# line/open-universe

Hardware: AMD Instinct MI355X
Metric: real_time_factor (audio s / wall s), UNIVERSE++ 16 kHz 8-step enhance (higher is better)
Workload: dtype f32; 1 GPU; UNIVERSE++ 16 kHz, 8 diffusion steps, batch=1 utterance(s) of 4 s per GPU per step; network=PP16, n_diffusion_steps=8, batch_per_gpu=1, samples_per_utterance=64000, launches_per_enhance=414

## Files before the change

open-universe_amd/csrc/ou_api.cpp:

```cpp
#include <hip/hip_runtime.h>

#include <cmath>
#include <cstdio>
#include <cstdlib>
#include <cstring>
#include <map>
#include <string>
#include <vector>

#include "../../include/ouniverse.h"
#include "../../include/ouniverse_tuning.h"
#include "ou_kernels.h"
#include "ou_model.h"

using namespace ou;

namespace {
thread_local std::string g_last_error;
constexpr int kMaxSteps = 256;
constexpr size_t kProfSlots = 32768;
constexpr float kInvSqrt2 = 0.70710678118654752440f;
constexpr size_t align256(size_t bytes) { return (bytes + 255) & ~size_t(255); }

struct TensorRef {
  size_t off;
  int C, T;
};
struct Options {
  int dbg = 0, xcd_map = -1, conv_direct = 5, fuse = -1, fuse_nc = 0, rate_small = 1, fuse_upfir = 1, block3 = 0, d4_fir = 1,
      d4_force = 0, d4_short = 1, d2_wk = 0, wino = 1, d2_map = -1, unfuse64 = 0, preact = 1;
  int gru_v = 2, gru_bmax = 0, gru_ts = 0, gru_upw = 0, gru_backoff = 0, gru_agent = -1, gru_dbg = 0;
  int split = -1;
  int dbg_dec0_under_gru = 0;
  int tile_prefetch = 1;
  int trace = 0, no_overlap = 0, ts = 0, deep_factor = 8, mask_fused = 1, split_wino = 1, d2_tile_rule = 1;
  int ens_share = 1;
  double tile_min = -1.0;
  std::string chain_ts;
};
}

struct ou_packer {
  Model m;
  std::map<std::string, HostTensor> sd;
  std::vector<float> blob;
  std::string err;
};

struct ou_handle {
  Model m;
  const float* W = nullptr;
  int device = 0;
  int num_cu = 256;
  std::string err;
  std::map<std::string, TensorRef> tensors;
  int n_launch = 0, n_conv = 0;
  int cond_B = 0, cond_T = 0;
  bool trace = false;
  Options opt;
  NormMode norm;
  std::string plan_with_options;
  int last_cfg = -1;
  long long* tstamps = nullptr;
  std::map<size_t, float> alphas;
  hipStream_t aux[3] = {nullptr, nullptr, nullptr};
  std::vector<hipEvent_t> events;
  size_t ev_used = 0;
  bool overlap = true;
  int force_cfg = -1, force_sc = 0;
  bool profile = false;
  struct ProfRec { double flops, bytes; int cfg; };
  std::vector<ProfRec> prof;
  size_t prof_used = 0;
  unsigned long long* prof_dev = nullptr;
  struct WsRec { const void* ws; size_t bytes; int B, T; };
  std::vector<WsRec> ws_ready;
  int gru_agent_stores = 0;
  int lanes = 1, lane = 0;
  int lane_max_b = 0;
  struct NoiseSource {
    bool on = false;
    unsigned long long seed = 0;
    std::vector<unsigned long long> streams;
    float* scratch = nullptr;
    size_t scratch_bytes = 0;
  } noise_src;
  double plane_per_sample = 0.0, wav_plane_per_sample = 0.0;
  bool ws_ok(const void* ws, size_t bytes, int B, int T) const {
    (void)T;
    for (const WsRec& r : ws_ready)
      if (r.ws == ws) return r.B == B && r.bytes <= bytes;
    return false;
  }
};

namespace {

int fail(ou_handle* h, int code, const std::string& msg) {
  if (h) h->err = msg;
  g_last_error = msg;
  return code;
}

struct Tensor {
  float* p = nullptr;
  int C = 0, T = 0;
};

struct OptDesc {
  const char* key;
  int Options::*ip;
  double Options::*dp;
  bool experiments_only;
  const char* doc;
};
const OptDesc kOptions[] = {
    {"conv_direct", &Options::conv_direct, nullptr, false, "kernel generations the conv launcher may use (0 .. 5, ConvArgs::direct)"},
    {"split", &Options::split, nullptr, false, "-1 rule / 0 never / 1 wherever possible: conv_split_kernel (bf16-split operands)"},
    {"split_wino", &Options::split_wino, nullptr, false, "experiments build: 0 = the plain bf16-split kernel also where its minimal-filtering form would take the layer"},
    {"wino", &Options::wino, nullptr, false, "0: never the minimal-filtering (Winograd / Cook-Toom) kernel variants"},
    {"fuse", &Options::fuse, nullptr, false, "-1 cost model / 0 never / 2 / 3: depth of the fused ConvBlock body (conv_chain kernels)"},
    {"fuse_nc", &Options::fuse_nc, nullptr, false, "128 / 256: columns per tile of the fused ConvBlock body (0: launcher's choice)"},
    {"fuse_upfir", &Options::fuse_upfir, nullptr, false, "0: up-path anti-alias FIR always as its own pass"},
    {"rate_small", &Options::rate_small, nullptr, false, "0: outermost rate-change convs on the generic kernels (no rate_down / rate_up)"},
    {"preact", &Options::preact, nullptr, false, "0: every PReLU in its consumer's operand path (ConvArgs::out_act never set)"},
    {"unfuse64", &Options::unfuse64, nullptr, false, "1: 64-channel ConvBlock bodies as three split-K launches"},
    {"block3", &Options::block3, nullptr, false, "1: the three body convs of a deep-level ConvBlock in one launch (experiments build only)"},
    {"xcd_map", &Options::xcd_map, nullptr, false, "block -> tile mapping of the LDS-tiled conv kernel (-1: launcher's choice)"},
    {"d2_map", &Options::d2_map, nullptr, false, "block -> tile mapping of the wide-load split-K kernels (-1: launcher's choice)"},
    {"d2_tile_rule", &Options::d2_tile_rule, nullptr, false, "0: round 5's 64- vs 32-column rule of the wide-load split-K kernels (ignores that only 64-column tiles have minimal filtering)"},
    {"d2_wk", &Options::d2_wk, nullptr, false, "4 / 8: K slices of conv_direct2_kernel (0: launcher's rule)"},
    {"d4_fir", &Options::d4_fir, nullptr, false, "0: up convs with a fusable FIR stay on the first-generation fused kernel"},
    {"d4_short", &Options::d4_short, nullptr, false, "0: the 401-frame levels at batch 1 stay on the first-generation kernels"},
    {"d4_force", &Options::d4_force, nullptr, false, "10 TM + log2(WK): that conv_direct4 tile shape wherever a layer admits it"},
    {"tile_min", nullptr, &Options::tile_min, false, "wave tiles per SIMD from which the no-split-K kernels take a layer (< 0: 1.2)"},
    {"tile_prefetch", &Options::tile_prefetch, nullptr, false, "0: no LDS prefetch of the epilogue operand in conv_direct3_kernel"},
    {"deep_factor", &Options::deep_factor, nullptr, false, "blocks of 64 x 128 per CU up to which a layer counts as 'deep' (split-K kernels)"},
    {"mask_fused", &Options::mask_fused, nullptr, false, "ragged batches: 0 = a separate tail-mask launch after EVERY producer (reference form of the masks)"},
    {"gru_v", &Options::gru_v, nullptr, false, "2 ring kernel / 1 polling-wave kernel (experiments build)"},
    {"gru_bmax", &Options::gru_bmax, nullptr, false, "cap on the utterances per GRU launch (forces the chunked path)"},
    {"gru_upw", &Options::gru_upw, nullptr, false, "hidden units per workgroup of the ring kernel (0: from the batch size)"},
    {"gru_backoff", &Options::gru_backoff, nullptr, false, "poll back-off experiments of the ring kernel (0: none)"},
    {"gru_agent_stores", &Options::gru_agent, nullptr, false, "-1 handle's mode / 0 plain / 1 agent-scope publishes"},
    {"gru_dbg", &Options::gru_dbg, nullptr, false, "bit 0 no republish safety net, bit 1 system-scope publishes, bit 2 FAULT INJECTION (tests)"},
    {"gru_ts", &Options::gru_ts, nullptr, false, "1: per-wave cycle stamps of the GRU kernel into the end of the workspace (tuning)"},
    {"ts", &Options::ts, nullptr, false, "1: per-wave phase stamps in ou_bench_conv (tuning)"},
    {"trace", &Options::trace, nullptr, false, "1: one line per conv launch on stderr"},
    {"no_overlap", &Options::no_overlap, nullptr, false, "1: no side streams inside a call (every kernel alone on the device)"},
    {"ens_share", &Options::ens_share, nullptr, false, "ou_enhance_ensemble: 1 = conditioner once over the B inputs, its results replicated; 0 = over all E * B rows"},
    {"dbg", &Options::dbg, nullptr, true, "phase ablation switches of the conv kernels: WRONG results by design"},
    {"dbg_dec0", &Options::dbg_dec0_under_gru, nullptr, true, "first decoder block under the GRU: upper-bound measurement, WRONG results"},
};
constexpr int kNumOptions = (int)(sizeof(kOptions) / sizeof(kOptions[0]));
const OptDesc* find_option(const char* key) {
  for (int i = 0; i < kNumOptions; i++)
    if (std::strcmp(kOptions[i].key, key) == 0) return &kOptions[i];
  return nullptr;
}

struct Runner {
  ou_handle* h;
  Options env;
  char* base;
  size_t cap;
  size_t off = 0;
  bool dry;
  hipStream_t st;
  hipStream_t main_st;
  int B;
  hipError_t herr = hipSuccess;
  bool oom = false;
  const char* where = "";
  size_t max_plane = 0;
  bool mel_scale_preset = false;
  bool ragged = false;
  const int* lens_dev = nullptr;
  const RowInfo* rows_dev = nullptr;
  LevelSpec lv;
  int level_T[kMaxLenLevels] = {0};
  unsigned* status_words = nullptr;
  unsigned long long* block3_bar = nullptr;
  int gru_area_rows = 0;
  bool gru_shared = false;

  Runner(ou_handle* h_, void* ws, size_t cap_, bool dry_, hipStream_t st_, int B_)
      : h(h_), env(h_->opt), base((char*)ws), cap(cap_), dry(dry_), st(st_), main_st(st_), B(B_) {
#ifndef OU_EXPERIMENTS
    env.dbg = 0; env.dbg_dec0_under_gru = 0;
#endif
  }
  static Runner conditioner_of(const Runner& r, int Bc) {
    Runner c(r.h, r.base, r.cap, false, r.st, Bc);
    c.status_words = r.status_words;
    c.block3_bar = r.block3_bar;
    c.gru_area_rows = r.B;
    c.off = r.off;
    c.mel_scale_preset = r.mel_scale_preset;
    c.lv = r.lv;
    for (int l = 0; l < kMaxLenLevels; l++) c.level_T[l] = r.level_T[l];
    return c;
  }
  void set_ragged(const int* lens, const RowInfo* rows) {
    ragged = true;
    lens_dev = lens;
    rows_dev = rows;
  }

  bool ok() const { return herr == hipSuccess && !oom; }
  template <class F>
  void launch(const char* w, F&& enqueue) {
    if (dry || !ok()) return;
    chk(enqueue(), w);
  }

  float* alloc_raw(size_t floats) {
// ... 2470 lines not shown
```

open-universe_amd/csrc/ou_conv_direct4.hip:

```cpp
#include "ou_kernels.h"
#include "ou_internal.h"
#include "ou_dev.h"

#include <cmath>
#include <cstdlib>
#include <type_traits>

namespace ou {

typedef float f32x4acc __attribute__((ext_vector_type(4)));

template <int R, int TM, int WN, int WK, int D>
__global__ __launch_bounds__(64 * WN * WK) void conv_direct4_kernel(ConvArgs p) {
  constexpr int TN = 4, LPS = 2 * R, BM = 16 * TM, NW = WN * WK, EP = 68;
  static_assert(WN == 1 || WK == 1, "a block is either WN column tiles or WK slices of the reduction");
  static_assert(TM >= 1 && TM <= 4, "16 .. 64-row tiles");
  static_assert(D * LPS <= 60, "loads in flight must fit vmcnt");
  static_assert(D == 2 || D == 4, "ring depth");
  typedef float f32x3 __attribute__((ext_vector_type(3)));
  typedef typename std::conditional<TM == 4, f32x4, typename std::conditional<TM == 3, f32x3,
          typename std::conditional<TM == 2, f32x2, float>::type>::type>::type avec;
  extern __shared__ __attribute__((aligned(16))) float smem[];
  const int tid = threadIdx.x, lane = tid & 63;
  const int wv = __builtin_amdgcn_readfirstlane(tid >> 6);
  const int wn = WK == 1 ? wv : 0, wk = WK == 1 ? 0 : wv;
  const int L = blockIdx.x, q8 = L >> 3;
  int rg, cidx;
  if (p.xcd_map == 1) {
    const int gm8 = (p.grid_m + 7) >> 3;
    rg = (q8 % gm8) * 8 + (L & 7);
    cidx = q8 / gm8;
  } else {
    rg = q8 % p.grid_m;
    cidx = (q8 / p.grid_m) * 8 + (L & 7);
  }
  const int b = cidx / p.grid_n, chunk = cidx - b * p.grid_n;
  const int n0 = (chunk * WN + wn) * 64, m0 = rg * BM;
  if (b >= p.B || rg >= p.grid_m) return;
  if (WK == 1 && n0 >= p.Nq) return;
  if (p.prof && tid == 0) atomicMin(p.prof + (blockIdx.x & 15), (unsigned long long)__builtin_amdgcn_s_memrealtime());
  const int l15 = lane & 15, kk = lane >> 4;
  const int Tin = p.Tin, Mp = p.Mp, CK = p.CK, lck = 31 - __clz(CK);
  const float alpha = p.act ? p.alpha_val : 1.0f;
  const u32x4 rx = direct_desc(p.x + (size_t)b * p.Cin * Tin, (unsigned)p.Cin * (unsigned)Tin * 4u);
  const u32x4 rw = direct_desc(p.w, (unsigned)p.Cin * (unsigned)R * (unsigned)Mp * 4u);
  const int avo = (kk * Mp + m0 + TM * l15) * 4;
  const int c0 = n0 + TN * l15;
  const int bvo = c0 < p.Nq ? (kk * Tin + c0 * R) * 4 : (int)0x80000000;

  const int NS = (p.Cin >> 2) / WK;
  avec a4[D][R];
  f32x4 b4[D][R];
#pragma unroll
  for (int d0 = 0; d0 < D; d0++)
#pragma unroll
    for (int k = 0; k < R; k++) {
      if constexpr (TM == 4) a4[d0][k] = f32x4{0.f, 0.f, 0.f, 0.f};
      else if constexpr (TM == 3) a4[d0][k] = f32x3{0.f, 0.f, 0.f};
      else if constexpr (TM == 2) a4[d0][k] = f32x2{0.f, 0.f};
      else a4[d0][k] = 0.f;
      b4[d0][k] = f32x4{0.f, 0.f, 0.f, 0.f};
    }
  f32x4acc acc[TM][TN];
#pragma unroll
  for (int i = 0; i < TM; i++)
#pragma unroll
    for (int j = 0; j < TN; j++) acc[i][j] = f32x4acc{0.f, 0.f, 0.f, 0.f};

#define OU_ISSUE(g_, d)                                                                                                  \
  {                                                                                                                      \
    const int c4 = (wk + WK * (g_)) * 4;                                                                                 \
    const int wrow = ((c4 >> lck) * R) * CK + (c4 & (CK - 1));                   \
    const int xso = c4 * Tin * 4;                                                                                        \
    _Pragma("unroll") for (int k = 0; k < R; k++) {                                                                      \
      if constexpr (TM == 4)                                                                                             \
        asm volatile("buffer_load_dwordx4 %0, %1, %2, %3 offen" : "+v"(a4[d][k]) : "v"(avo), "s"(rw), "s"((wrow + k * CK) * Mp * 4)); \
      else if constexpr (TM == 3)                                                                                        \
        asm volatile("buffer_load_dwordx3 %0, %1, %2, %3 offen" : "+v"(a4[d][k]) : "v"(avo), "s"(rw), "s"((wrow + k * CK) * Mp * 4)); \
      else if constexpr (TM == 2)                                                                                        \
        asm volatile("buffer_load_dwordx2 %0, %1, %2, %3 offen" : "+v"(a4[d][k]) : "v"(avo), "s"(rw), "s"((wrow + k * CK) * Mp * 4)); \
      else                                                                                                               \
        asm volatile("buffer_load_dword %0, %1, %2, %3 offen" : "+v"(a4[d][k]) : "v"(avo), "s"(rw), "s"((wrow + k * CK) * Mp * 4)); \
    }                                                                                                                    \
    _Pragma("unroll") for (int k = 0; k < R; k++)                                                                        \
      asm volatile("buffer_load_dwordx4 %0, %1, %2, %3 offen offset:%4" : "+v"(b4[d][k]) : "v"(bvo), "s"(rx), "s"(xso), "n"(16 * k)); \
  }
#define OU_MMA(d, out)                                                                                                   \
  {                                                                                                                      \
    asm volatile("s_waitcnt vmcnt(%0)" ::"n"((out) * LPS));                                                              \
    _Pragma("unroll") for (int k = 0; k < R; k++) { asm volatile("" : "+v"(a4[d][k])); asm volatile("" : "+v"(b4[d][k])); } \
    float X[4 * R];                                                                                                      \
    _Pragma("unroll") for (int k = 0; k < R; k++) {                                                                      \
      X[4 * k + 0] = b4[d][k].x; X[4 * k + 1] = b4[d][k].y; X[4 * k + 2] = b4[d][k].z; X[4 * k + 3] = b4[d][k].w;        \
    }                                                                                                                    \
    _Pragma("unroll") for (int e = 0; e < 4 * R; e++) X[e] = X[e] >= 0.f ? X[e] : alpha * X[e];                          \
    _Pragma("unroll") for (int k = 0; k < R; k++)                                                                        \
      _Pragma("unroll") for (int i = 0; i < TM; i++) {                                                                   \
        float av;                                                                                                        \
        if constexpr (TM == 1) av = a4[d][k]; else av = a4[d][k][i];                                                     \
        _Pragma("unroll") for (int j = 0; j < TN; j++)                                                                   \
          acc[i][j] = __builtin_amdgcn_mfma_f32_16x16x4f32(av, X[j * R + k], acc[i][j], 0, 0, 0);                        \
      }                                                                                                                  \
  }
  const bool ts_on = p.tstamps != nullptr;
  long long tc0 = 0, tc1 = 0, tc2 = 0, tr0 = 0;
  if (ts_on) { tr0 = (long long)__builtin_amdgcn_s_memrealtime(); tc0 = __builtin_readcyclecounter(); }
  if constexpr (D == 4) {
    OU_ISSUE(0, 0); OU_ISSUE(1, 1); OU_ISSUE(2, 2); OU_ISSUE(3, 3);
    if (ts_on) tc1 = __builtin_readcyclecounter();
    const int NR = NS / 4;
    for (int r = 0; r + 1 < NR; r++) {
      const int g = r * 4;
      OU_MMA(0, 3); OU_ISSUE(g + 4, 0);
      OU_MMA(1, 3); OU_ISSUE(g + 5, 1);
      OU_MMA(2, 3); OU_ISSUE(g + 6, 2);
      OU_MMA(3, 3); OU_ISSUE(g + 7, 3);
    }
    OU_MMA(0, 3); OU_MMA(1, 2); OU_MMA(2, 1); OU_MMA(3, 0);
  } else {
    OU_ISSUE(0, 0); OU_ISSUE(1, 1);
    if (ts_on) tc1 = __builtin_readcyclecounter();
    const int NR = NS / 2;
    for (int r = 0; r + 1 < NR; r++) {
      const int g = r * 2;
      OU_MMA(0, 1); OU_ISSUE(g + 2, 0);
      OU_MMA(1, 1); OU_ISSUE(g + 3, 1);
    }
    OU_MMA(0, 1); OU_MMA(1, 0);
  }
  if (ts_on) tc2 = __builtin_readcyclecounter();
#undef OU_ISSUE
#undef OU_MMA

  float* Ew = smem + (size_t)wv * BM * EP;
#pragma unroll
  for (int i = 0; i < TM; i++)
#pragma unroll
    for (int r = 0; r < 4; r++)
      *reinterpret_cast<f32x4*>(&Ew[(TM * (4 * kk + r) + i) * EP + 4 * l15]) =
          f32x4{acc[i][0][r], acc[i][1][r], acc[i][2][r], acc[i][3][r]};
  if constexpr (WK > 1) asm volatile("s_waitcnt lgkmcnt(0)\n\ts_barrier" ::: "memory");
  else asm volatile("s_waitcnt lgkmcnt(0)" ::: "memory");

  const int rt = WK == 1 ? lane : tid;
  constexpr int RNT = WK == 1 ? 64 : 64 * WK;
  const float* Er = WK == 1 ? Ew : smem;
  const float* filmb = p.film ? p.film + (size_t)b * p.film_bstride : nullptr;
  const size_t ybase = (size_t)b * p.Cout * p.Tout;
  const float insc = p.in_scale ? p.in_scale[b] : 1.0f;
  const int nvalid = p.Nq - n0;
  const int rlen = ragged_len(p.lens, b);
  if (p.up == 1) {
    constexpr int NQ = BM * 16, QPT = (NQ + RNT - 1) / RNT;
#pragma unroll
    for (int u = 0; u < QPT; u++) {
      const int e = rt + u * RNT;
      if (NQ % RNT != 0 && e >= NQ) break;
      const int row = e >> 4, cq = (e & 15) * 4;
      const int m = m0 + row;
      if (m >= p.M || cq >= nvalid) continue;
      const size_t idx = ybase + (size_t)m * p.Tout + n0 + cq;
      const bool full = cq + 4 <= nvalid;
      f32x4 ad = {0.f, 0.f, 0.f, 0.f}, rs = {0.f, 0.f, 0.f, 0.f};
      if (full) {
        if (p.add) ad = *reinterpret_cast<const f32x4u*>(p.add + idx);
        if (p.res) rs = *reinterpret_cast<const f32x4u*>(p.res + idx);
      } else {
#pragma unroll
        for (int s = 0; s < 4; s++) {
          if (p.add && cq + s < nvalid) ad[s] = p.add[idx + s];
          if (p.res && cq + s < nvalid) rs[s] = p.res[idx + s];
        }
      }
      f32x4 v = *reinterpret_cast<const f32x4*>(&Er[row * EP + cq]);
#pragma unroll
      for (int k = 1; k < WK; k++) v += *reinterpret_cast<const f32x4*>(&Er[(k * BM + row) * EP + cq]);
      if (p.in_scale) v *= insc;
      v += p.bias[m];
      if (p.add) v = (v + ad) * p.add_scale;
      if (filmb) v = filmb[m] * v + filmb[p.Cout + m];
      if (p.res) v = (v + rs) * p.res_scale;
      if (p.lens) v = ragged_mask4(v, n0 + cq, rlen);
      if (full) {
        *reinterpret_cast<f32x4u*>(p.y + idx) = v;
      } else {
#pragma unroll
        for (int s = 0; s < 4; s++)
          if (cq + s < nvalid) p.y[idx + s] = v[s];
      }
    }
  } else {
    const int up = p.up;
    const int m_hi = (m0 + BM - 1 < p.M - 1) ? m0 + BM - 1 : p.M - 1;
    const int co_lo = (int)__umulhi((unsigned)m0, p.magic_up);
    const int nco = (int)__umulhi((unsigned)m_hi, p.magic_up) - co_lo + 1;
    const int qpc = 16 * up;
    const int total = nco * qpc;
    for (int e = rt; e < total; e += RNT) {
      const int cl = (int)__umulhi((unsigned)(e >> 4), p.magic_up);
      const int tl = (e - cl * qpc) * 4;
      const int co = co_lo + cl;
      const int q0 = (int)__umulhi((unsigned)tl, p.magic_up);
      int ph = tl - q0 * up, q = q0;
      f32x4 v;
      bool ok[4];
#pragma unroll
      for (int s = 0; s < 4; s++) {
        const int row = co * up + ph - m0;
        ok[s] = row >= 0 && row < BM && m0 + row <= m_hi && q < nvalid;
        float a = 0.f;
        if (ok[s]) {
          a = Er[row * EP + q];
#pragma unroll
          for (int k = 1; k < WK; k++) a += Er[(k * BM + row) * EP + q];
        }
        v[s] = a;
        if (++ph == up) { ph = 0; q++; }
      }
      const size_t idx = ybase + (size_t)co * p.Tout + (size_t)n0 * up + tl;
      const bool full = ok[0] && ok[1] && ok[2] && ok[3];
      if (!(ok[0] || ok[1] || ok[2] || ok[3])) continue;
      f32x4 ad = {0.f, 0.f, 0.f, 0.f}, rs = {0.f, 0.f, 0.f, 0.f};
      if (full) {
        if (p.add) ad = *reinterpret_cast<const f32x4u*>(p.add + idx);
        if (p.res) rs = *reinterpret_cast<const f32x4u*>(p.res + idx);
      } else {
#pragma unroll
        for (int s = 0; s < 4; s++) {
          if (p.add && ok[s]) ad[s] = p.add[idx + s];
          if (p.res && ok[s]) rs[s] = p.res[idx + s];
        }
      }
      if (p.in_scale) v *= insc;
      v += p.bias[co];
      if (p.add) v = (v + ad) * p.add_scale;
// ... 185 lines not shown
      for (int s = 0; s < 4; s++) {
        if (p.add && cq + s < nvalid) ad[s] = p.add[idx + s];
        if (p.res && cq + s < nvalid) rs[s] = p.res[idx + s];
      }
    }
    f32x4 v = *reinterpret_cast<const f32x4*>(&smem[row * EP + cq]);
#pragma unroll
    for (int k = 1; k < WK; k++) v += *reinterpret_cast<const f32x4*>(&smem[(k * BM + row) * EP + cq]);
    if (p.in_scale) v *= insc;
    v += p.bias[m];
    if (p.add) v = (v + ad) * p.add_scale;
    if (filmb) v = filmb[m] * v + filmb[p.Cout + m];
    if (p.res) v = (v + rs) * p.res_scale;
    if (p.out_act) {
#pragma unroll
      for (int s = 0; s < 4; s++) v[s] = v[s] >= 0.f ? v[s] : p.out_alpha * v[s];
    }
    if (p.lens) v = ragged_mask4(v, n0 + cq, ragged_len(p.lens, b));
    if (full) {
      *reinterpret_cast<f32x4u*>(p.y + idx) = v;
    } else {
#pragma unroll
      for (int s = 0; s < 4; s++)
        if (cq + s < nvalid) p.y[idx + s] = v[s];
    }
  }
  if (ts_on && lane == 0) {
    const long long tc5 = __builtin_readcyclecounter();
    long long* o = p.tstamps + ((size_t)blockIdx.x * WK + wk) * 8;
    o[0] = tr0; o[1] = tc1 - tc0; o[2] = tc2 - tc1; o[3] = tc3 - tc2; o[4] = tc4 - tc3; o[5] = tc5 - tc4; o[6] = twait;
    o[7] = (long long)__builtin_amdgcn_s_memrealtime();
  }
  if (p.prof && tid == 0) atomicMin(p.prof + 16 + (blockIdx.x & 15), ~(unsigned long long)__builtin_amdgcn_s_memrealtime());
}

struct Direct4wCfg {
  int KW, TM, WK;
  void (*kern)(ConvArgs);
};
#define OU_D4W(KW, TM, WK) {KW, TM, WK, conv_direct4w_kernel<KW, TM, WK>}
static const Direct4wCfg kDirect4wCfgs[] = {OU_D4W(3, 1, 8), OU_D4W(3, 2, 8), OU_D4W(5, 1, 8), OU_D4W(5, 2, 8),
                                            OU_D4W(3, 1, 4), OU_D4W(3, 2, 4), OU_D4W(5, 1, 4), OU_D4W(5, 2, 4)};
hipError_t launch_conv_direct4w(const ConvArgs& a, int num_cu, hipStream_t stream, int* cfg_out) {
  if (!a.wu || a.stride != 1 || a.up != 1 || (a.KW != 3 && a.KW != 5) || a.pad != (a.KW - 1) / 2 || a.fir || a.Cin % 16 ||
      (a.in_scale != nullptr && a.act))
    return hipErrorInvalidConfiguration;
  if ((long)a.Cin * a.Tin * 4 >= (1L << 31) || (long)a.Cin * a.Mp * 8 * 4 >= (1L << 31)) return hipErrorInvalidConfiguration;
  const bool forced = a.force_cfg >= 600 && a.force_cfg < 800;
  if (!forced && !(a.wino && a.direct >= 5)) return hipErrorInvalidConfiguration;
  const int slots = a.Cin / 4;
  const long ct = (a.Nq + 63) / 64;
  int tm = 0, wk = 8;
  if (forced) {
    tm = ((a.force_cfg % 100) / 10);
    wk = a.force_cfg >= 700 ? 4 : 8;
  } else {
    const long b64 = (long)((a.M + 31) / 32) * ct * a.B;
    if (a.Nq >= 1024 || b64 * 10 >= (long)num_cu * 8) return hipErrorInvalidConfiguration;
    long best = 0;
    for (int t = 1; t <= 2; t++) {
      const long blocks = (long)((a.M + 16 * t - 1) / (16 * t)) * ct * a.B;
      const long cost = (blocks + num_cu - 1) / num_cu * t;
      if (!tm || cost <= best) { tm = t; best = cost; }
    }
  }
  if (tm < 1 || tm > 2 || slots % (wk * 4) != 0) return hipErrorInvalidConfiguration;
  const Direct4wCfg* c = nullptr;
  for (const Direct4wCfg& k : kDirect4wCfgs)
    if (k.KW == a.KW && k.TM == tm && k.WK == wk) { c = &k; break; }
  if (!c) return hipErrorInvalidConfiguration;
  ConvArgs aa = a;
  const long gy = (a.M + 16 * tm - 1) / (16 * tm);
  aa.grid_m = (int)gy;
  aa.grid_n = (int)ct;
  const long nblocks = 8L * ((gy + 7) / 8) * ct * a.B;
  if (cfg_out) *cfg_out = (wk == 4 ? 700 : 600) + 10 * tm + a.KW;
  hipLaunchKernelGGL(c->kern, dim3((unsigned)nblocks), dim3(64 * wk), (size_t)wk * 16 * tm * 68 * 4, stream, aa);
  return hipGetLastError();
}

struct Direct4Cfg {
  int R, TM, WN, WK, D;
  void (*kern)(ConvArgs);
};
#define OU_D4(R, TM, WN, WK, D) {R, TM, WN, WK, D, conv_direct4_kernel<R, TM, WN, WK, D>}
#ifdef OU_EXPERIMENTS
#define OU_D4_SHAPES(R, D)                                                                                    \
  OU_D4(R, 4, 4, 1, D), OU_D4(R, 2, 4, 1, D), OU_D4(R, 4, 1, 2, D), OU_D4(R, 2, 1, 2, D), OU_D4(R, 4, 1, 4, D), \
  OU_D4(R, 2, 1, 4, D), OU_D4(R, 4, 1, 8, D), OU_D4(R, 2, 1, 8, D), OU_D4(R, 1, 1, 4, D), OU_D4(R, 1, 1, 8, D), \
  OU_D4(R, 3, 1, 4, D), OU_D4(R, 3, 1, 8, D)
#else
#define OU_D4_SHAPES(R, D)                                                                            \
  OU_D4(R, 2, 4, 1, D), OU_D4(R, 2, 1, 2, D), OU_D4(R, 2, 1, 4, D), OU_D4(R, 2, 1, 8, D), OU_D4(R, 1, 1, 4, D), \
  OU_D4(R, 1, 1, 8, D), OU_D4(R, 3, 1, 4, D), OU_D4(R, 3, 1, 8, D)
#endif
static const Direct4Cfg kDirect4Cfgs[] = {
    OU_D4_SHAPES(1, 4), OU_D4_SHAPES(2, 4), OU_D4_SHAPES(3, 2), OU_D4_SHAPES(4, 2), OU_D4_SHAPES(5, 2), OU_D4_SHAPES(8, 2),
};
static size_t direct4_smem(const Direct4Cfg& c) { return (size_t)c.WN * c.WK * 16 * c.TM * 68 * 4; }
hipError_t init_direct4_kernels() {
  for (const Direct4Cfg& c : kDirect4Cfgs) {
    if (direct4_smem(c) <= 64 * 1024) continue;
    hipError_t e = hipFuncSetAttribute(reinterpret_cast<const void*>(c.kern), hipFuncAttributeMaxDynamicSharedMemorySize,
                                       (int)direct4_smem(c));
    if (e != hipSuccess) return e;
  }
  return hipSuccess;
}

static bool direct4_pick(int M, long ct_b, int slots, int R, int D, bool short_layer, int num_cu, int* tm_out, int* wk_out) {
  if (short_layer) {
    int wk = 8;
    while (wk > 4 && slots % (wk * D) != 0) wk >>= 1;
    if (slots % (wk * D)) return false;
    int best_tm = 0;
    long best_cost = 0;
    for (int tm = 1; tm <= 3; tm++) {
      const long blocks = (long)((M + 16 * tm - 1) / (16 * tm)) * ct_b;
      const long cost = (blocks + num_cu - 1) / num_cu * tm;
      if (!best_tm || cost <= best_cost) { best_tm = tm; best_cost = cost; }
    }
    *tm_out = best_tm; *wk_out = wk;
    return true;
  }
  const long tiles = (long)((M + 31) / 32) * ct_b;
  int wk = 8;
  while (wk > 1 && (slots % (wk * D) != 0 || (slots / wk) * 8 * R < 64 || tiles * wk > 12000)) wk >>= 1;
  if (slots % (wk * D)) return false;
  *tm_out = 2; *wk_out = wk;
  return true;
}

hipError_t launch_conv_direct4(const ConvArgs& a, int num_cu, hipStream_t stream, int* cfg_out, bool probe) {
  const int R = a.stride > 1 ? a.stride : 1;
  if (a.KW != R || a.pad != 0 || (a.stride > 1 && (a.up != 1 || a.Tin != a.Nq * R)) || a.Cin % 16 || a.CK % 4 || a.fir ||
      (a.in_scale != nullptr && a.act))
    return hipErrorInvalidConfiguration;
  if ((long)a.Cin * a.Tin * 4 >= (1L << 31) || (long)a.Cin * a.KW * a.Mp * 4 >= (1L << 31)) return hipErrorInvalidConfiguration;
  if (a.up > 1 && (a.Cout * a.up != a.M || a.Tout != a.Nq * a.up)) return hipErrorInvalidConfiguration;
  const int slots = a.Cin / 4;
  const long ct = (a.Nq + 63) / 64;
  const bool short_layer = a.Nq < 1024 && a.B < 4;
  if (a.force_cfg < 300 && a.d4_force == 0 && short_layer && (!a.d4_short || a.B > 1 || (probe && a.up > 1)))
    return hipErrorInvalidConfiguration;
  const Direct4Cfg* best = nullptr;
  auto code = [](const Direct4Cfg& c) { return 10 * c.TM + (c.WK == 1 ? 0 : c.WK == 2 ? 1 : c.WK == 4 ? 2 : 3); };
  const int D = R <= 2 ? 4 : 2;
  int want = a.force_cfg >= 300 ? a.force_cfg - 300 : a.d4_force;
  for (int pass = 0; pass < 2 && !best; pass++) {
    if (pass == 1) {
      if (a.force_cfg >= 300) break;
      int tm = 0, wk = 0;
      if (!direct4_pick(a.M, ct * a.B, slots, R, D, short_layer, num_cu, &tm, &wk)) break;
      want = 10 * tm + (wk == 1 ? 0 : wk == 2 ? 1 : wk == 4 ? 2 : 3);
    } else if (want == 0) {
      continue;
    }
    for (const Direct4Cfg& c : kDirect4Cfgs)
      if (c.R == R && slots % (c.WK * c.D) == 0 && code(c) == want) { best = &c; break; }
  }
  if (!best) return hipErrorInvalidConfiguration;
  if (a.out_act) return hipErrorNotSupported;
  if (probe) return hipSuccess;
  const Direct4Cfg& c = *best;
  ConvArgs aa = a;
  const long gy = (a.M + 16 * c.TM - 1) / (16 * c.TM);
  aa.grid_m = (int)gy;
  aa.magic_up = a.up == 1 ? 0u : (unsigned)(0x100000000ull / (unsigned)a.up) + 1u;
  const long chunks = (ct + c.WN - 1) / c.WN;
  aa.grid_n = (int)chunks;
  const double xb = (double)a.Cin * a.Tin * a.B, wb = (double)a.M * a.Cin * a.KW;
  aa.xcd_map = wb > xb ? 1 : 2;
  if (a.force_xcd_map == 1 || a.force_xcd_map == 2) aa.xcd_map = a.force_xcd_map;
  const long nblocks = aa.xcd_map == 1 ? 8L * ((gy + 7) / 8) * chunks * a.B : (chunks * a.B + 7) / 8 * 8 * gy;
  if (cfg_out) *cfg_out = 300 + code(c);
  hipLaunchKernelGGL(c.kern, dim3((unsigned)nblocks), dim3(64 * c.WN * c.WK), direct4_smem(c), stream, aa);
  return hipGetLastError();
}

}
```

open-universe_amd/csrc/ou_conv_mfma.hip:

```cpp
#include "ou_kernels.h"
#include "ou_internal.h"
#include "ou_dev.h"

#include <cmath>
#include <cstdlib>
#include <type_traits>

namespace ou {

constexpr int CONV_XCAP = 4096;
constexpr int CONV_XCAP_BIG = 8192;

template <int TM, int TN, int WM, int WN, int WK, int CONV_MAXW, int U, bool EXACT>
__global__ __launch_bounds__(64 * WM * WN * WK) void conv_mfma_kernel(ConvArgs p) {
  constexpr int CONV_NT = 64 * WM * WN * WK;
  constexpr int XCAP = (WK == 8 && TM * TN == 4) ? CONV_XCAP_BIG : CONV_XCAP;
  constexpr int CONV_MAXX = XCAP / CONV_NT;
  static_assert(WM * WN * WK == 4 || WM * WN * WK == 8, "4 or 8 waves per block");
  constexpr int BM = 32 * TM * WM, BN = 32 * TN * WN;
  extern __shared__ __attribute__((aligned(16))) float smem[];

  const int tid = threadIdx.x, lane = tid & 63;
  const int wave = __builtin_amdgcn_readfirstlane(tid >> 6);
  const int kw = wave % WK, wn = (wave / WK) % WN, wm = wave / (WK * WN);
// ... 332 lines not shown
    o[4] = __builtin_readcyclecounter() - tsv[4]; o[5] = t_mma; o[6] = t_wait; o[7] = tsv[0];
  }
}

struct ConvCfg {
  int BM, BN, WK, MAXW, NT, XCAP;
  void (*kern4)(ConvArgs);
  void (*kern2)(ConvArgs);
  void (*kern_g)(ConvArgs);
};
#define OU_CONV_CFG(BM, BN, WK, MAXW, NT, TM, TN, WM, WN)                                             \
  {BM, BN, WK, MAXW, NT, (WK == 8 && TM * TN == 4) ? CONV_XCAP_BIG : CONV_XCAP,                       \
   conv_mfma_kernel<TM, TN, WM, WN, WK, MAXW, 4, true>,                          \
   conv_mfma_kernel<TM, TN, WM, WN, WK, MAXW, 2, true>, conv_mfma_kernel<TM, TN, WM, WN, WK, MAXW, 2, false>}
#define OU_CONV_CFG_OFF(BM, BN, WK, MAXW, NT) {BM, BN, WK, MAXW, NT, CONV_XCAP, nullptr, nullptr, nullptr}
static const ConvCfg kConvCfgs[] = {
    OU_CONV_CFG(64, 128, 1, 6, 256, 1, 2, 2, 2),
    OU_CONV_CFG(32, 128, 1, 6, 256, 1, 1, 1, 4),
    OU_CONV_CFG(64, 64, 1, 6, 256, 1, 1, 2, 2),
#ifdef OU_EXPERIMENTS
    OU_CONV_CFG(32, 64, 4, 12, 256, 1, 2, 1, 1),
    OU_CONV_CFG(32, 32, 4, 12, 256, 1, 1, 1, 1),
#else
    OU_CONV_CFG_OFF(32, 64, 4, 12, 256), OU_CONV_CFG_OFF(32, 32, 4, 12, 256),
#endif
    OU_CONV_CFG(32, 64, 8, 6, 512, 1, 2, 1, 1),
    OU_CONV_CFG(32, 32, 8, 6, 512, 1, 1, 1, 1),
#ifdef OU_EXPERIMENTS
    OU_CONV_CFG(64, 64, 8, 12, 512, 2, 2, 1, 1),
#else
    OU_CONV_CFG_OFF(64, 64, 8, 12, 512),
#endif
};
constexpr int kNumConvCfgs = sizeof(kConvCfgs) / sizeof(kConvCfgs[0]);

static size_t conv_smem_bytes(const ConvCfg& c, const ConvArgs& a) {
  int span = (c.BN - 1) * a.stride + a.KW;
  size_t xt_al = ((size_t)a.SC * a.CK * span + 3) & ~size_t(3);
  size_t stage = 2 * (xt_al + (size_t)a.SC * a.CK * a.KW * c.BM) + 2 * c.BM;
  if (c.WK == 8) stage += 2 * 4 * c.WK;
  size_t epi = (size_t)c.WK * c.BM * (c.BN + 4);
  return 4 * (stage > epi ? stage : epi);
}

hipError_t init_conv_kernels() {
  hipError_t e_d3 = hipSuccess;
  for (int i = 0; i < kNumConvCfgs; i++) {
    if (!kConvCfgs[i].kern4) continue;
    hipError_t e = hipFuncSetAttribute(reinterpret_cast<const void*>(kConvCfgs[i].kern4),
                                       hipFuncAttributeMaxDynamicSharedMemorySize, 160 * 1024);
    if (e != hipSuccess) return e;
    e = hipFuncSetAttribute(reinterpret_cast<const void*>(kConvCfgs[i].kern2),
                            hipFuncAttributeMaxDynamicSharedMemorySize, 160 * 1024);
    if (e != hipSuccess) return e;
    e = hipFuncSetAttribute(reinterpret_cast<const void*>(kConvCfgs[i].kern_g),
                            hipFuncAttributeMaxDynamicSharedMemorySize, 160 * 1024);
    if (e != hipSuccess) return e;
  }
  e_d3 = init_direct3_kernels();
  if (e_d3 != hipSuccess) return e_d3;
  e_d3 = init_block3_kernels();
  if (e_d3 != hipSuccess) return e_d3;
  e_d3 = init_direct4_kernels();
  if (e_d3 != hipSuccess) return e_d3;
  e_d3 = init_split_kernels();
  if (e_d3 != hipSuccess) return e_d3;
  return init_chain_kernels();
}

bool conv_masks_rows(int cfg) { return cfg >= 0 && !(cfg >= 100 && cfg < 200); }

namespace {
hipError_t try_split(const ConvArgs& a, int num_cu, hipStream_t stream, int* cfg_out) {
  if (!a.wsplit || a.split == 0) return hipErrorInvalidConfiguration;
  const double tiles = (double)(a.M / 64) * ((a.Nq + 127) / 128) * a.B / 4.0;
  const bool rule = a.M >= 256 && a.M % 256 == 0 && tiles >= ((a.Nq < 1024 || a.KW == 5) ? 0.45 : 0.9) * num_cu;
  if (!(a.split == 1 || a.force_cfg >= 800 || rule)) return hipErrorInvalidConfiguration;
  return launch_conv_split(a, num_cu, stream, cfg_out);
}
hipError_t try_direct3(const ConvArgs& a, int num_cu, hipStream_t stream, int* cfg_out) {
  if (a.direct < 3) return hipErrorInvalidConfiguration;
  return launch_conv_direct3(a, num_cu, stream, cfg_out);
}
hipError_t try_direct4(const ConvArgs& a, int num_cu, hipStream_t stream, int* cfg_out) {
  if (a.direct < 4) return hipErrorInvalidConfiguration;
  if (a.fir) {
    if (a.d4_fir_unfused && a.force_cfg < 0) {
      ConvArgs probe = a;
      probe.fir = nullptr; probe.fir_len = 0;
      if (launch_conv_direct4(probe, num_cu, stream, nullptr, true) == hipSuccess) return hipErrorNotSupported;
    }
    return a.force_cfg >= 0 ? hipErrorNotSupported : hipErrorInvalidConfiguration;
  }
  return launch_conv_direct4(a, num_cu, stream, cfg_out, false);
}
hipError_t try_direct4w(const ConvArgs& a, int num_cu, hipStream_t stream, int* cfg_out) {
  if (a.direct < 5) return hipErrorInvalidConfiguration;
  return launch_conv_direct4w(a, num_cu, stream, cfg_out);
}
hipError_t try_direct(const ConvArgs& a, int num_cu, hipStream_t stream, int* cfg_out) {
  if (a.direct == 0) return hipErrorInvalidConfiguration;
  const long wide = (long)((a.M + 63) / 64) * ((a.Nq + 127) / 128) * a.B;
  const bool wide_ok = a.wd && a.direct >= 2 && a.stride == 1 && a.up == 1;
  const bool deep = ((a.Nq <= 16384 || wide_ok) && wide < (long)a.deep_factor * num_cu) || a.force_cfg >= 100;
  if (!deep) return hipErrorInvalidConfiguration;
  return launch_conv_direct(a, num_cu, stream, cfg_out);
}
struct ConvFamily {
  int lo, hi;
  bool final_if_forced;
  hipError_t (*attempt)(const ConvArgs&, int, hipStream_t, int*);
};
const ConvFamily kConvFamilies[] = {
    {800, 1100, true, try_split},
    {200, 300, true, try_direct3},
    {300, 500, true, try_direct4},
    {600, 800, true, try_direct4w},
    {100, 200, false, try_direct},
};
bool forced_into(const ConvFamily& f, int cfg) {
  if (cfg >= f.lo && cfg < f.hi) return true;
  return f.attempt == try_direct3 && cfg >= 500 && cfg < 600;
}
}

hipError_t launch_conv(const ConvArgs& a, int num_cu, hipStream_t stream, int* cfg_out) {
  if (a.Cin % a.CK || a.CK < 2 || (a.CK & (a.CK - 1)) || a.Mp % 64 || a.Nq <= 0) return hipErrorInvalidValue;
  for (const ConvFamily& f : kConvFamilies) {
    const bool forced = a.force_cfg >= 0 && forced_into(f, a.force_cfg);
    if (a.force_cfg >= 0 && !forced) continue;
    const hipError_t e = f.attempt(a, num_cu, stream, cfg_out);
    if (e != hipErrorInvalidConfiguration) return e;
    if (forced && f.final_if_forced) return e;
  }
  if (a.fir) return hipErrorNotSupported;
  int pick = -1;
  for (int i = 0; i < kNumConvCfgs; i++) {
    const ConvCfg& c = kConvCfgs[i];
    if (a.force_cfg >= 0 && i != a.force_cfg) continue;
    if (!c.kern4) continue;
    if (c.BM == 64 && a.M <= 32) continue;
    int span = (c.BN - 1) * a.stride + a.KW;
    if ((long)a.CK * span > c.XCAP) continue;
    if ((long)a.CK * a.KW * c.BM > (long)c.MAXW * c.NT * 4) continue;
    if (a.force_cfg < 0 && c.WK == 4) continue;
    if (a.force_cfg < 0 && c.BM == 64 && c.WK == 8) continue;
    if (a.force_cfg < 0 && c.WK == 1 && a.KW > 1 && a.Nq < 1024 && a.Cin * a.KW >= 1024) continue;
    if (a.force_cfg < 0 && c.WK == 8 && c.BN == 64 && a.stride >= 4 &&
        (long)((a.M + c.BM - 1) / c.BM) * ((a.Nq + c.BN - 1) / c.BN) * a.B < 2L * num_cu)
      continue;
    if (a.force_cfg < 0 && c.WK == 8 && c.BN == 64 && a.KW == 1 && a.Nq < 1024) continue;
    pick = i;
    const long want = c.WK == 1 ? (long)num_cu * 3 / 2 : (long)num_cu * 15 / 16;
    long blocks = (long)((a.M + c.BM - 1) / c.BM) * ((a.Nq + c.BN - 1) / c.BN) * a.B;
    if (blocks >= want) break;
  }
  if (pick < 0) return hipErrorInvalidConfiguration;
  if (a.out_act) return hipErrorNotSupported;
  const ConvCfg& c = kConvCfgs[pick];
  if (cfg_out) *cfg_out = pick;
  ConvArgs aa = a;
  {
    const int span = (c.BN - 1) * a.stride + a.KW;
    const int nch = a.Cin / a.CK;
    int sc = 1;
    for (int cand = 4; cand >= 2; cand >>= 1) {
      if (a.force_sc > 0 && cand > a.force_sc) continue;
      if (nch % cand) continue;
      if ((long)cand * a.CK * span > c.XCAP) continue;
      if ((long)cand * a.CK * a.KW * c.BM > (long)c.MAXW * c.NT * 4) continue;
      aa.SC = cand;
      if (conv_smem_bytes(c, aa) > 160 * 1024) continue;
      sc = cand;
      break;
    }
// ... 29 lines not shown
```

open-universe_amd/csrc/ou_kernels.h:

```cpp
#pragma once
#include <hip/hip_runtime.h>

#include <cstddef>
#include <cstdint>

namespace ou {

struct ConvArgs {
  const float* x = nullptr;
  const float* w = nullptr;
  const float* wd = nullptr;
  const float* wu = nullptr;
  const void* wsplit = nullptr;
  const void* wsplitw = nullptr;
  int split_wino = 1;
  const float* bias = nullptr;
  float* y = nullptr;
  const float* in_scale = nullptr;
  int act = 0;
  float alpha_val = 0.f;
  const float* add = nullptr;
  const float* film = nullptr;
  const float* res = nullptr;
  float add_scale = 1.f, res_scale = 1.f;
  int film_bstride = 0;
  int B = 1, Cin = 0, Tin = 0, Cout = 0, M = 0, Mp = 0, KW = 1, stride = 1, pad = 0, up = 1, CK = 2;
  int Nq = 0;
  int Tout = 0;
  unsigned magic_span[3] = {0, 0, 0};
  unsigned magic_up = 0;
  int SC = 1;
  int grid_n = 1, grid_m = 1;
  int xcd_map = 0;
  int force_cfg = -1, force_sc = 0;
  int force_xcd_map = -1;
  double tile_min = -1.0;
  int tile_prefetch = 1;
  int direct = 5;
  int d2_map = -1;
  int split = -1;
  int wino = 1;
  int d2_wk = 0;
  int d4_fir_unfused = 1;
  int d4_short = 1;
  int d4_force = 0;
  int d2_tile_rule = 1;
  int deep_factor = 8;
  int out_act = 0;
  float out_alpha = 1.f;
  const int* lens = nullptr;
  const float* fir = nullptr;
  int fir_len = 0;
  int tile_bm = 32, tile_bn = 0, tile_halo = 0;
  int dbg = 0;
  long long* tstamps = nullptr;
  unsigned long long* prof = nullptr;
};
hipError_t launch_conv(const ConvArgs& a, int num_cu, hipStream_t stream, int* cfg_out = nullptr);
bool conv_masks_rows(int cfg);
hipError_t init_conv_kernels();
double direct3_tiles_per_simd(int M, int Nq, int B, int num_cu);
bool rate_down_supported(const ConvArgs& a);
hipError_t launch_rate_down(const ConvArgs& a, hipStream_t st, int* cfg_out = nullptr);
bool rate_up_supported(const ConvArgs& a);
hipError_t launch_rate_up(const ConvArgs& a, hipStream_t st, int* cfg_out = nullptr);

struct StepCoef {
  float w_in, sigma_net, w_skip, w_out, sig2, c1, s_next, beta;
};
enum OutMode { OUT_SCORE = 0, OUT_UPDATE = 1 };
hipError_t launch_in_conv(const float* x, const float* w, const float* bias, const StepCoef* coef, int coef_bstride,
                          float* y, int B, int C, int T, int KW, hipStream_t s, const int* lens = nullptr);
hipError_t launch_out_conv(const float* s, const float* w, const float* bias, const float* alphas, const float* x,
                           const float* noise, float* out, const StepCoef* coef, int coef_bstride, int edm,
                           int mode, int B, int C, int T, int KW, hipStream_t st, const int* lens = nullptr);

hipError_t launch_sigma_embed(const StepCoef* coef, int S, const float* params, int simple, int n_rff, int D,
                              float* g, hipStream_t st);
hipError_t launch_film(const float* g, const float* W, const float* b, float* film, int S, int rows, int D,
                       hipStream_t st);
struct CoefBlock { StepCoef c[64]; };
hipError_t launch_upload_coef(StepCoef* dst, const CoefBlock& blk, int n, hipStream_t st);

struct RowInfo { int t_raw, pad_left, t_pad, _r; };
struct NormMode {
  int norm = 0;
  int zero_mean = 1;
  float eps = 1e-5f;
  bool plain() const { return norm == 0 && zero_mean; }
  __host__ __device__ float gain(float level, float sd, float mx) const {
    if (norm == 1) return level / fmaxf(mx, eps);
    if (norm == 2) return fminf(level / fmaxf(sd, eps), 1.f / fmaxf(mx, eps));
    return level / fmaxf(sd, eps);
  }
};
constexpr int kMaxLenLevels = 8;
struct LevelSpec { int n = 0; int num[kMaxLenLevels]; int den[kMaxLenLevels]; };
struct RowBlock { int t_raw[64]; };
hipError_t launch_upload_rows(RowInfo* rows, int* lens, const RowBlock& blk, int n, int off, int B, int tot_ds,
                              const LevelSpec& lv, hipStream_t st);
hipError_t launch_mask_tail(float* y, const int* lens, int B, int C, int T, hipStream_t st);
hipError_t launch_gru_tail_fill(float* gx, const int* lens, int B, int H, int T, hipStream_t st);
hipError_t launch_pad_normalize_var(const float* mix, float* y, float* stats, const RowInfo* rows, int B, int T_raw_max,
                                    int T_pad_max, float level, const NormMode& nm, hipStream_t st);
hipError_t launch_post_var(const float* x, const float* stats, float* out, const RowInfo* rows, int B, int T_raw_max,
                           int T_pad_max, int keep_rms, int peak_guard, hipStream_t st);

hipError_t launch_pad_normalize(const float* mix, float* y, float* stats, int B, int T_raw, int T_pad, int pad_left,
                                float level, const NormMode& nm, hipStream_t st);
hipError_t launch_post(const float* x, const float* stats, float* out, int B, int T_raw, int T_pad, int pad_left,
                       int keep_rms, int peak_guard, hipStream_t st);
hipError_t launch_init_x(const float* noise, const float* base, float sigma, float* x, size_t n, hipStream_t st);

hipError_t launch_sampler_step(float* x, const float* score, const float* z, float c1, float c2, size_t n,
                               hipStream_t st);

hipError_t launch_stft_forward(const float* x, const float* win, float* out, int B, int T, int n_fft, int hop,
                               int type, float e, float factor, hipStream_t st);
hipError_t launch_stft_inverse(const float* spec, const float* win, float* frames, float* y, int B, int n_frames,
                               int n_fft, int hop, int type, float e, float factor, int length, hipStream_t st);

hipError_t launch_mel(const float* x, const float* win, const float* tw, const float* fb, float* mel, float* esum,
                      int B, int T, int n_fft, int hop, int pad_left, int n_freq, int n_mels, int L, hipStream_t st);
hipError_t launch_mel_scale(const float* esum, float* scale, int B, int L, hipStream_t st, const int* lens = nullptr);

struct SegGeom {
// ... 194 lines not shown
```

Measured before the change: 616.5 x_realtime.

## Fuse anti-alias FIR epilogue into conv_direct4 up-conv kernel by launcher rule

Adds a FIR-epilogue variant of conv_direct4_kernel for upsampling convs (up 4/5). It uses overlapping 62-column tiles with a one-column halo so the polyphase FIR, bias, residual and mask are applied in LDS before the store. This avoids a separate FIR pass and the write and reread of the intermediate upsampled tensor. The new default applies it at batch 1 for large outputs. In exchange, tiles overlap by two columns, so some GEMM work is recomputed and the epilogue costs more registers.

```diff
diff --git a/open-universe_amd/csrc/ou_api.cpp b/open-universe_amd/csrc/ou_api.cpp
--- a/open-universe_amd/csrc/ou_api.cpp
+++ b/open-universe_amd/csrc/ou_api.cpp
@@ -27,7 +27,7 @@
   int C, T;
 };
 struct Options {
-  int dbg = 0, xcd_map = -1, conv_direct = 5, fuse = -1, fuse_nc = 0, rate_small = 1, fuse_upfir = 1, block3 = 0, d4_fir = 1,
+  int dbg = 0, xcd_map = -1, conv_direct = 5, fuse = -1, fuse_nc = 0, rate_small = 1, fuse_upfir = 1, block3 = 0, d4_fir = 2,
       d4_force = 0, d4_short = 1, d2_wk = 0, wino = 1, d2_map = -1, unfuse64 = 0, preact = 1;
   int gru_v = 2, gru_bmax = 0, gru_ts = 0, gru_upw = 0, gru_backoff = 0, gru_agent = -1, gru_dbg = 0;
   int split = -1;
@@ -130,7 +130,7 @@
     {"d2_map", &Options::d2_map, nullptr, false, "block -> tile mapping of the wide-load split-K kernels (-1: launcher's choice)"},
     {"d2_tile_rule", &Options::d2_tile_rule, nullptr, false, "0: round 5's 64- vs 32-column rule of the wide-load split-K kernels (ignores that only 64-column tiles have minimal filtering)"},
     {"d2_wk", &Options::d2_wk, nullptr, false, "4 / 8: K slices of conv_direct2_kernel (0: launcher's rule)"},
-    {"d4_fir", &Options::d4_fir, nullptr, false, "0: up convs with a fusable FIR stay on the first-generation fused kernel"},
+    {"d4_fir", &Options::d4_fir, nullptr, false, "up convs with a fusable FIR: 0 stay on the first-generation fused kernel, 1 conv_direct4_kernel + FIR pass, 2 its FIR epilogue by the launcher's rule, 3 wherever supported"},
     {"d4_short", &Options::d4_short, nullptr, false, "0: the 401-frame levels at batch 1 stay on the first-generation kernels"},
     {"d4_force", &Options::d4_force, nullptr, false, "10 TM + log2(WK): that conv_direct4 tile shape wherever a layer admits it"},
     {"tile_min", nullptr, &Options::tile_min, false, "wave tiles per SIMD from which the no-split-K kernels take a layer (< 0: 1.2)"},
diff --git a/open-universe_amd/csrc/ou_conv_direct4.hip b/open-universe_amd/csrc/ou_conv_direct4.hip
--- a/open-universe_amd/csrc/ou_conv_direct4.hip
+++ b/open-universe_amd/csrc/ou_conv_direct4.hip
@@ -10,9 +10,11 @@
 
 typedef float f32x4acc __attribute__((ext_vector_type(4)));
 
-template <int R, int TM, int WN, int WK, int D>
+template <int R, int TM, int WN, int WK, int D, bool FIR = false>
 __global__ __launch_bounds__(64 * WN * WK) void conv_direct4_kernel(ConvArgs p) {
   constexpr int TN = 4, LPS = 2 * R, BM = 16 * TM, NW = WN * WK, EP = 68;
+  constexpr int ADV = FIR ? 62 : 64;
+  static_assert(!FIR || R == 1, "the FIR epilogue belongs to the phase GEMMs");
   static_assert(WN == 1 || WK == 1, "a block is either WN column tiles or WK slices of the reduction");
   static_assert(TM >= 1 && TM <= 4, "16 .. 64-row tiles");
   static_assert(D * LPS <= 60, "loads in flight must fit vmcnt");
@@ -35,18 +37,19 @@
     cidx = (q8 / p.grid_m) * 8 + (L & 7);
   }
   const int b = cidx / p.grid_n, chunk = cidx - b * p.grid_n;
-  const int n0 = (chunk * WN + wn) * 64, m0 = rg * BM;
+  const int n0 = (chunk * WN + wn) * ADV - (FIR ? 1 : 0), m0 = rg * (FIR ? p.tile_bm : BM);
   if (b >= p.B || rg >= p.grid_m) return;
-  if (WK == 1 && n0 >= p.Nq) return;
+  if (WK == 1 && n0 + (FIR ? 1 : 0) >= p.Nq) return;
   if (p.prof && tid == 0) atomicMin(p.prof + (blockIdx.x & 15), (unsigned long long)__builtin_amdgcn_s_memrealtime());
   const int l15 = lane & 15, kk = lane >> 4;
   const int Tin = p.Tin, Mp = p.Mp, CK = p.CK, lck = 31 - __clz(CK);
   const float alpha = p.act ? p.alpha_val : 1.0f;
-  const u32x4 rx = direct_desc(p.x + (size_t)b * p.Cin * Tin, (unsigned)p.Cin * (unsigned)Tin * 4u);
+  constexpr int XS = FIR ? 1 : 0;
+  const u32x4 rx = direct_desc(p.x + (size_t)b * p.Cin * Tin - XS, ((unsigned)p.Cin * (unsigned)Tin + XS) * 4u);
   const u32x4 rw = direct_desc(p.w, (unsigned)p.Cin * (unsigned)R * (unsigned)Mp * 4u);
   const int avo = (kk * Mp + m0 + TM * l15) * 4;
   const int c0 = n0 + TN * l15;
-  const int bvo = c0 < p.Nq ? (kk * Tin + c0 * R) * 4 : (int)0x80000000;
+  const int bvo = c0 < p.Nq ? (kk * Tin + c0 * R + XS) * 4 : (int)0x80000000;
 
   const int NS = (p.Cin >> 2) / WK;
   avec a4[D][R];
@@ -150,7 +153,85 @@
   const float insc = p.in_scale ? p.in_scale[b] : 1.0f;
   const int nvalid = p.Nq - n0;
   const int rlen = ragged_len(p.lens, b);
-  if (p.up == 1) {
+  if constexpr (FIR) {
+    float* E0 = WK == 1 ? Ew : smem;
+    auto fir_epi = [&](auto up_c) __attribute__((always_inline)) {
+      constexpr int UP = decltype(up_c)::value, NTP = 2 * UP + 1, WIN = NTP + 3, SPAN = ADV * UP, QPC = (SPAN + 3) / 4, NCO = BM / UP;
+      float f[NTP];
+#pragma unroll
+      for (int j = 0; j < NTP; j++) f[j] = p.fir[j];
+      const int co_lo = m0 / UP;
+      const int tbase = (n0 + 1) * UP;
+      const int tlim = rlen < p.Tout ? rlen : p.Tout;
+      constexpr int FQ = (NCO * QPC + RNT - 1) / RNT;
+      f32x4 rsv[FQ];
+#pragma unroll
+      for (int u = 0; u < FQ; u++) {
+        const int e = rt + u * RNT;
+        const int cl = e / QPC, tl = (e - cl * QPC) * 4, co = co_lo + cl, t = tbase + tl;
+        rsv[u] = f32x4{0.f, 0.f, 0.f, 0.f};
+        if (p.res && e < NCO * QPC && co < p.Cout && tl + 3 < SPAN && t + 3 < p.Tout)
+          rsv[u] = *reinterpret_cast<const f32x4u*>(p.res + ybase + (size_t)co * p.Tout + t);
+      }
+      if constexpr (WK > 1) {
+        constexpr int NQ = BM * 16;
+        for (int e = tid; e < NQ; e += RNT) {
+          const int row = e >> 4, cq = (e & 15) * 4;
+          f32x4 v = *reinterpret_cast<const f32x4*>(&smem[row * EP + cq]);
+#pragma unroll
+          for (int k = 1; k < WK; k++) v += *reinterpret_cast<const f32x4*>(&smem[(k * BM + row) * EP + cq]);
+          *reinterpret_cast<f32x4*>(&smem[row * EP + cq]) = v;
+        }
+        asm volatile("s_waitcnt lgkmcnt(0)\n\ts_barrier" ::: "memory");
+      }
+#pragma unroll
+      for (int u = 0; u < FQ; u++) {
+        const int e = rt + u * RNT;
+        if (e >= NCO * QPC) break;
+        const int cl = e / QPC, tl = (e - cl * QPC) * 4, co = co_lo + cl, t = tbase + tl;
+        if (co >= p.Cout || t >= p.Tout) continue;
+        int q = tl / UP, ph = tl - q * UP;
+        float w[WIN];
+#pragma unroll
+        for (int i = 0; i < WIN; i++) {
+          const int tt = t - UP + i;
+          const float a = E0[(cl * UP + ph) * EP + q];
+          w[i] = (tt >= 0 && tt < tlim) ? a : 0.f;
+          if (++ph == UP) { ph = 0; q++; }
+        }
+        bool ok[4];
+#pragma unroll
+        for (int s = 0; s < 4; s++) ok[s] = tl + s < SPAN && t + s < p.Tout;
+        const bool full = ok[0] && ok[1] && ok[2] && ok[3];
+        const size_t idx = ybase + (size_t)co * p.Tout + t;
+        f32x4 rs = rsv[u];
+        if (p.res && !full) {
+#pragma unroll
+          for (int s = 0; s < 4; s++) if (ok[s]) rs[s] = p.res[idx + s];
+        }
+        const float bb = p.bias[co];
+        f32x4 o;
+#pragma unroll
+        for (int s = 0; s < 4; s++) {
+          float acc = 0.f;
+#pragma unroll
+          for (int j = 0; j < NTP; j++) acc = fmaf(f[j], w[s + j], acc);
+          acc += bb;
+          if (p.res) acc = (acc + rs[s]) * p.res_scale;
+          o[s] = acc;
+        }
+        if (p.lens) o = ragged_mask4(o, t, rlen);
+        if (full) {
+          *reinterpret_cast<f32x4u*>(p.y + idx) = o;
+        } else {
+#pragma unroll
+          for (int s = 0; s < 4; s++) if (ok[s]) p.y[idx + s] = o[s];
+        }
+      }
+    };
+    if (p.up == 4) fir_epi(std::integral_constant<int, 4>{});
+    else fir_epi(std::integral_constant<int, 5>{});
+  } else if (p.up == 1) {
     constexpr int NQ = BM * 16, QPT = (NQ + RNT - 1) / RNT;
 #pragma unroll
     for (int u = 0; u < QPT; u++) {
@@ -502,8 +583,14 @@
 struct Direct4Cfg {
   int R, TM, WN, WK, D;
   void (*kern)(ConvArgs);
+  void (*kern_fir)(ConvArgs);
 };
-#define OU_D4(R, TM, WN, WK, D) {R, TM, WN, WK, D, conv_direct4_kernel<R, TM, WN, WK, D>}
+template <int R, int TM, int WN, int WK, int D>
+constexpr auto direct4_fir_kernel() -> void (*)(ConvArgs) {
+  if constexpr (R == 1 && TM <= 3) return conv_direct4_kernel<R, TM, WN, WK, D, true>;
+  else return nullptr;
+}
+#define OU_D4(R, TM, WN, WK, D) {R, TM, WN, WK, D, conv_direct4_kernel<R, TM, WN, WK, D>, direct4_fir_kernel<R, TM, WN, WK, D>()}
 #ifdef OU_EXPERIMENTS
 #define OU_D4_SHAPES(R, D)                                                                                    \
   OU_D4(R, 4, 4, 1, D), OU_D4(R, 2, 4, 1, D), OU_D4(R, 4, 1, 2, D), OU_D4(R, 2, 1, 2, D), OU_D4(R, 4, 1, 4, D), \
@@ -524,6 +611,9 @@
     hipError_t e = hipFuncSetAttribute(reinterpret_cast<const void*>(c.kern), hipFuncAttributeMaxDynamicSharedMemorySize,
                                        (int)direct4_smem(c));
     if (e != hipSuccess) return e;
+    if (!c.kern_fir) continue;
+    e = hipFuncSetAttribute(reinterpret_cast<const void*>(c.kern_fir), hipFuncAttributeMaxDynamicSharedMemorySize, (int)direct4_smem(c));
+    if (e != hipSuccess) return e;
   }
   return hipSuccess;
 }
@@ -553,15 +643,19 @@
 
 hipError_t launch_conv_direct4(const ConvArgs& a, int num_cu, hipStream_t stream, int* cfg_out, bool probe) {
   const int R = a.stride > 1 ? a.stride : 1;
-  if (a.KW != R || a.pad != 0 || (a.stride > 1 && (a.up != 1 || a.Tin != a.Nq * R)) || a.Cin % 16 || a.CK % 4 || a.fir ||
+  if (a.KW != R || a.pad != 0 || (a.stride > 1 && (a.up != 1 || a.Tin != a.Nq * R)) || a.Cin % 16 || a.CK % 4 ||
       (a.in_scale != nullptr && a.act))
+    return hipErrorInvalidConfiguration;
+  const bool fir = a.fir != nullptr;
+  if (fir && (R != 1 || (a.up != 4 && a.up != 5) || a.fir_len != 2 * a.up + 1 || a.add || a.film || a.in_scale || a.out_act))
     return hipErrorInvalidConfiguration;
   if ((long)a.Cin * a.Tin * 4 >= (1L << 31) || (long)a.Cin * a.KW * a.Mp * 4 >= (1L << 31)) return hipErrorInvalidConfiguration;
   if (a.up > 1 && (a.Cout * a.up != a.M || a.Tout != a.Nq * a.up)) return hipErrorInvalidConfiguration;
   const int slots = a.Cin / 4;
-  const long ct = (a.Nq + 63) / 64;
+  const long ct = fir ? (a.Nq + 61) / 62 : (a.Nq + 63) / 64;
   const bool short_layer = a.Nq < 1024 && a.B < 4;
-  if (a.force_cfg < 300 && a.d4_force == 0 && short_layer && (!a.d4_short || a.B > 1 || (probe && a.up > 1)))
+  if (a.force_cfg < 300 && a.d4_force == 0 && short_layer && !(fir && a.d4_fir_unfused >= 3) &&
+      (!a.d4_short || a.B > 1 || (probe && a.up > 1)))
     return hipErrorInvalidConfiguration;
   const Direct4Cfg* best = nullptr;
   auto code = [](const Direct4Cfg& c) { return 10 * c.TM + (c.WK == 1 ? 0 : c.WK == 2 ? 1 : c.WK == 4 ? 2 : 3); };
@@ -577,15 +671,17 @@
       continue;
     }
     for (const Direct4Cfg& c : kDirect4Cfgs)
-      if (c.R == R && slots % (c.WK * c.D) == 0 && code(c) == want) { best = &c; break; }
+      if (c.R == R && slots % (c.WK * c.D) == 0 && code(c) == want && (!fir || c.kern_fir)) { best = &c; break; }
   }
   if (!best) return hipErrorInvalidConfiguration;
   if (a.out_act) return hipErrorNotSupported;
   if (probe) return hipSuccess;
   const Direct4Cfg& c = *best;
   ConvArgs aa = a;
-  const long gy = (a.M + 16 * c.TM - 1) / (16 * c.TM);
+  const int bmu = fir ? 16 * c.TM / a.up * a.up : 16 * c.TM;
+  const long gy = (a.M + bmu - 1) / bmu;
   aa.grid_m = (int)gy;
+  aa.tile_bm = bmu;
   aa.magic_up = a.up == 1 ? 0u : (unsigned)(0x100000000ull / (unsigned)a.up) + 1u;
   const long chunks = (ct + c.WN - 1) / c.WN;
   aa.grid_n = (int)chunks;
@@ -594,7 +690,7 @@
   if (a.force_xcd_map == 1 || a.force_xcd_map == 2) aa.xcd_map = a.force_xcd_map;
   const long nblocks = aa.xcd_map == 1 ? 8L * ((gy + 7) / 8) * chunks * a.B : (chunks * a.B + 7) / 8 * 8 * gy;
   if (cfg_out) *cfg_out = 300 + code(c);
-  hipLaunchKernelGGL(c.kern, dim3((unsigned)nblocks), dim3(64 * c.WN * c.WK), direct4_smem(c), stream, aa);
+  hipLaunchKernelGGL(fir ? c.kern_fir : c.kern, dim3((unsigned)nblocks), dim3(64 * c.WN * c.WK), direct4_smem(c), stream, aa);
   return hipGetLastError();
 }
 
diff --git a/open-universe_amd/csrc/ou_conv_mfma.hip b/open-universe_amd/csrc/ou_conv_mfma.hip
--- a/open-universe_amd/csrc/ou_conv_mfma.hip
+++ b/open-universe_amd/csrc/ou_conv_mfma.hip
@@ -438,15 +438,27 @@
   if (a.direct < 3) return hipErrorInvalidConfiguration;
   return launch_conv_direct3(a, num_cu, stream, cfg_out);
 }
+bool direct4_fir_rule(const ConvArgs& a) { return a.B == 1 && (size_t)a.Cout * a.Tout * 4 >= ((size_t)2 << 20); }
 hipError_t try_direct4(const ConvArgs& a, int num_cu, hipStream_t stream, int* cfg_out) {
   if (a.direct < 4) return hipErrorInvalidConfiguration;
   if (a.fir) {
-    if (a.d4_fir_unfused && a.force_cfg < 0) {
-      ConvArgs probe = a;
-      probe.fir = nullptr; probe.fir_len = 0;
-      if (launch_conv_direct4(probe, num_cu, stream, nullptr, true) == hipSuccess) return hipErrorNotSupported;
-    }
-    return a.force_cfg >= 0 ? hipErrorNotSupported : hipErrorInvalidConfiguration;
+    if (a.force_cfg >= 0) {
+      const hipError_t e = launch_conv_direct4(a, num_cu, stream, cfg_out, false);
+      return e == hipErrorInvalidConfiguration ? hipErrorNotSupported : e;
+    }
+    if (a.d4_fir_unfused == 0) return hipErrorInvalidConfiguration;
+    if (a.d4_fir_unfused >= 3) {
+      const hipError_t e = launch_conv_direct4(a, num_cu, stream, cfg_out, false);
+      if (e != hipErrorInvalidConfiguration) return e;
+    }
+    ConvArgs probe = a;
+    probe.fir = nullptr; probe.fir_len = 0;
+    if (launch_conv_direct4(probe, num_cu, stream, nullptr, true) != hipSuccess) return hipErrorInvalidConfiguration;
+    if (a.d4_fir_unfused >= 2 && direct4_fir_rule(a)) {
+      const hipError_t e = launch_conv_direct4(a, num_cu, stream, cfg_out, false);
+      if (e != hipErrorInvalidConfiguration) return e;
+    }
+    return hipErrorNotSupported;
   }
   return launch_conv_direct4(a, num_cu, stream, cfg_out, false);
 }
diff --git a/open-universe_amd/csrc/ou_kernels.h b/open-universe_amd/csrc/ou_kernels.h
--- a/open-universe_amd/csrc/ou_kernels.h
+++ b/open-universe_amd/csrc/ou_kernels.h
@@ -41,7 +41,7 @@
   int split = -1;
   int wino = 1;
   int d2_wk = 0;
-  int d4_fir_unfused = 1;
+  int d4_fir_unfused = 2;
   int d4_short = 1;
   int d4_force = 0;
   int d2_tile_rule = 1;
```

New measurement: 614.0 x_realtime, median of 2. About the same (-0.4%).
